# IrisRainbowNeko/HCP-Diffusion

Measured on AMD Instinct MI355X. Metric: training images/sec (whole node), SD1.5 LoRA 512px bs=4/GPU, higher is better.
Workload: dtype bf16; 1 GPU; SD1.5 UNet LoRA rank=8 bf16, bs=4/GPU, 512x512 (64x64 latents), 77-token context, random-init weights, cached latents, grad-ckpt off; global_batch=4, parallelism=dp1, rccl_ranks=1, comm=none, hip_graph=True, gradient_checkpointing=False

## Files before the change

hcp_diffusion_amd/csrc/gemm.hip:

```cpp
#include "hcp_common.h"
#include "gemm_params.h"

extern "C" int hcp_geglu_fwd(const void* h, void* y, long M, int F, hipStream_t stream);

namespace {

using namespace hcp_gemm;


HCP_DEVICE void epilogue_store(const GemmParams& p, int m, int n, hcp_f32x4 v) {
    if (p.geglu_hg) { epilogue_geglu_bwd(p, m, n, v); return; }
    v = v * p.alpha;
    if (p.bias) v += *(const hcp_f32x4*)(p.bias + n);
    if (p.rowbias) v += *(const hcp_f32x4*)(p.rowbias + (size_t)(m / p.rows_per_group) * p.rowbias_ld + n);
    if (p.residual) {
        hcp_bf16x4 r = *(const hcp_bf16x4*)(p.residual + (size_t)m * p.ldr + n);
#pragma unroll
        for (int q = 0; q < 4; ++q) v[q] += hcp_bf2f((unsigned short)r[q]);
        add_residual_lo(p, m, n, v);
    }
    if (p.out_f32) *(hcp_f32x4*)((float*)p.D + (size_t)m * p.ldd + n) = v;
    else store_hi_lo(p, m, n, v);
}

// ... 744 lines not shown
            const hcp_f32x4 a = *(const hcp_f32x4*)(src + (size_t)s * slab), b = *(const hcp_f32x4*)(src + (size_t)(s + 1) * slab);
            v += a; v += b;
            s += 2;
        }
        if (s < ns) v += *(const hcp_f32x4*)(src + (size_t)s * slab);
        if (!plain) { epilogue_geglu_bwd(p, m, n, v); continue; }
        v = v * p.alpha;
        if (p.bias) v += bias;
        if (p.rowbias) v += rowb;
        if (p.residual) {
#pragma unroll
            for (int q = 0; q < 4; ++q) v[q] += hcp_bf2f((unsigned short)res[q]);
            if (p.residual_lo) {
#pragma unroll
                for (int q = 0; q < 4; ++q) v[q] += hcp_bf2f((unsigned short)res_lo[q]);
            }
        }
        if (p.out_f32) *(hcp_f32x4*)((float*)p.D + (size_t)m * p.ldd + n) = v;
        else store_hi_lo(p, m, n, v);
    }
}

HCP_TUNABLE(int, g_force_cfg, -1);
HCP_TUNABLE(int, g_dbg_ablate, 0);
HCP_TUNABLE(int, g_use_glds, 1);
HCP_TUNABLE(int, g_use_v2, 1);

HCP_TUNABLE(int, g_conv_patch, 1);
HCP_TUNABLE(int, g_epi_tile, -1);
HCP_TUNABLE(int, g_force_loaders, -1);

bool want_epi_tile(const GemmParams& p, int mode) {
    if (p.nsplit != 1 || p.out_f32 || p.geglu_hg || p.geglu_out || p.N % 8 || p.ldd % 8 || (p.residual && p.ldr % 8)) return false;
    if ((((size_t)p.D) | ((size_t)p.D_lo) | ((size_t)p.residual) | ((size_t)p.residual_lo)) & 15) return false;
    if (g_epi_tile >= 0) return g_epi_tile == 1;
    return mode == 0 && p.residual != nullptr;
}

template <int BM, int BN, int WGM, int WGN, int MODE, bool FAST, bool LORA = false, int NSTAGE = 2, int NLD = 0>
int launch_cfg(GemmParams& p, hipStream_t stream) {
    p.tiles_m = hcp_cdiv(p.M, BM);
    const int tiles_n = hcp_cdiv(p.N, BN);
    p.dbg = g_dbg_ablate;
    if constexpr (NSTAGE == 2 && (MODE == 0 || FAST)) {
        if (g_use_v2 && g_use_glds && !(p.dbg & 7) && p.K % BK == 0 && (p.K2 == 0 || p.K2 == 32) &&
            (size_t)p.M * p.lda * 2 < (1ul << 31) && (size_t)p.N * p.ldb * 2 < (1ul << 31)) {
// ... 32 lines not shown
            HCP_LAUNCH_CHECK("gemm_v2_kernel");
        }
    }
    {
        p.epi_tile = 0;
        p.geglu_out = nullptr;
        size_t smem = (size_t)NSTAGE * (BM + BN + (LORA ? 32 : 0)) * BK * sizeof(hcp_bf16);
        const size_t tail = (size_t)(2 * BM + BN) * 40 * sizeof(hcp_bf16);
        if (LORA && smem < tail) smem = tail;
        HCP_LAUNCH((gemm_glds_kernel<BM, BN, WGM, WGN, MODE, FAST, LORA, NSTAGE>), dim3(p.tiles_m * tiles_n, p.nsplit),
                   dim3(64 * WGM * WGN), smem, stream, p);
    }
    if (p.nsplit > 1) {
        long nv = (long)p.M * (p.N / 4);
        int g = (int)((nv + 255) / 256); if (g > 2048) g = 2048;
        HCP_LAUNCH(splitk_reduce_kernel, dim3(g), dim3(256), 0, stream, p);
    }
    HCP_LAUNCH_CHECK("gemm_kernel");
}

struct TileCfg { int bm, bn; };
constexpr TileCfg kCfgs[] = {{128, 128}, {128, 64}, {64, 64}, {128, 160}, {64, 160}, {256, 128}, {256, 160}, {128, 320},
                             {128, 160}, {128, 160}, {256, 160},
                             {128, 320}, {256, 160}, {128, 160}, {64, 160}, {128, 128}};
constexpr int kNumCfgs = sizeof(kCfgs) / sizeof(kCfgs[0]);

int try_pp(int id, int mode, bool fast_or_plain, bool lora, GemmParams& p, hipStream_t stream) {
    if (p.loaders < 8 || !fast_or_plain || !g_use_v2 || (g_dbg_ablate & 7)) return -2;
    if (p.K % BK != 0 || !(p.K2 == 0 || p.K2 == 32) || (size_t)p.M * p.lda * 2 >= (1ul << 31) || (size_t)p.N * p.ldb * 2 >= (1ul << 31)) return -2;
    const int bm = kCfgs[id].bm, bn = kCfgs[id].bn;
    p.tiles_m = hcp_cdiv(p.M, bm);
    p.dbg = g_dbg_ablate;
    p.epi_tile = want_epi_tile(p, mode) ? 1 : 0;
    hcp_bf16* const gout = p.geglu_out;
    if (gout) {
        if (mode == 0 && p.nsplit == 1 && (p.N / 2) % (bn / 2) == 0) p.geglu_fused = 1;
        else p.geglu_out = nullptr;
    }
    int r = -2;
    if (mode != 0 && !lora && (g_conv_patch == 2 || (g_conv_patch == 1 && (mode == 2 || p.nsplit > 1))))
        r = conv_patch_launch(p, bm, bn, mode, p.loaders - 8, stream);
    if (r == -2) r = gemm_pp_launch(p, bm, bn, mode, lora, p.loaders - 8, stream);
    if (r == -2) { p.geglu_out = gout; p.geglu_fused = 0; }
    if (r != 0 || p.nsplit <= 1) return r;
    long nv = (long)p.M * (p.N / 4);
    int g = (int)((nv + 255) / 256); if (g > 2048) g = 2048;
    HCP_LAUNCH(splitk_reduce_kernel, dim3(g), dim3(256), 0, stream, p);
    HCP_LAUNCH_CHECK("splitk_reduce_kernel");
}

template <int MODE, bool FAST>
int launch_by_id(int id, GemmParams& p, hipStream_t stream) {
    if (id >= 0 && id < kNumCfgs) { const int r = try_pp(id, MODE, MODE == 0 || FAST, false, p, stream); if (r != -2) return r; }
    switch (id) {
        case 0: return launch_cfg<128, 128, 2, 2, MODE, FAST>(p, stream);
        case 1: return launch_cfg<128, 64, 2, 2, MODE, FAST>(p, stream);
        case 2: return launch_cfg<64, 64, 2, 2, MODE, FAST>(p, stream);
        case 3: return launch_cfg<128, 160, 2, 2, MODE, FAST>(p, stream);
        case 4: return launch_cfg<64, 160, 2, 2, MODE, FAST>(p, stream);
        case 5: return launch_cfg<256, 128, 4, 2, MODE, FAST>(p, stream);
        case 6: return launch_cfg<256, 160, 4, 2, MODE, FAST>(p, stream);
        case 8: return launch_cfg<128, 160, 4, 2, MODE, FAST, false, 3>(p, stream);
        case 9: return launch_cfg<128, 160, 2, 2, MODE, FAST, false, 3>(p, stream);
        case 10: return launch_cfg<256, 160, 4, 2, MODE, FAST, false, 3>(p, stream);
        case 11: return launch_cfg<128, 320, 4, 4, MODE, FAST>(p, stream);
        case 12: return launch_cfg<256, 160, 8, 2, MODE, FAST>(p, stream);
        case 13: return launch_cfg<128, 160, 4, 2, MODE, FAST, false, 2, 4>(p, stream);
        case 14: return launch_cfg<64, 160, 4, 2, MODE, FAST, false, 2, 4>(p, stream);
        case 15: return launch_cfg<128, 128, 4, 2, MODE, FAST, false, 2, 4>(p, stream);
        default: return launch_cfg<128, 320, 2, 4, MODE, FAST>(p, stream);
    }
}

int launch_lora_by_id(int id, GemmParams& p, hipStream_t stream) {
    if (id >= 0 && id < kNumCfgs) { const int r = try_pp(id, 0, true, true, p, stream); if (r != -2) return r; }
    switch (id) {
        case 0: return launch_cfg<128, 128, 2, 2, 0, false, true>(p, stream);
        case 1: return launch_cfg<128, 64, 2, 2, 0, false, true>(p, stream);
        case 2: return launch_cfg<64, 64, 2, 2, 0, false, true>(p, stream);
        case 3: return launch_cfg<128, 160, 2, 2, 0, false, true>(p, stream);
        case 5: return launch_cfg<256, 128, 4, 2, 0, false, true>(p, stream);
        case 6: return launch_cfg<256, 160, 4, 2, 0, false, true>(p, stream);
        case 8: return launch_cfg<128, 160, 4, 2, 0, false, true, 3>(p, stream);
        case 9: return launch_cfg<128, 160, 2, 2, 0, false, true, 3>(p, stream);
        case 12: return launch_cfg<256, 160, 8, 2, 0, false, true>(p, stream);
        case 13: return launch_cfg<128, 160, 4, 2, 0, false, true, 2, 4>(p, stream);
        case 14: return launch_cfg<64, 160, 4, 2, 0, false, true, 2, 4>(p, stream);
        case 15: return launch_cfg<128, 128, 4, 2, 0, false, true, 2, 4>(p, stream);
        default: return launch_cfg<64, 160, 2, 2, 0, false, true>(p, stream);
    }
}

int choose_cfg(const GemmParams& p, int* nsplit_out) {
    const int nk1 = hcp_cdiv(p.K, BK);
    int id;
    if (p.N <= 64) id = 2;
    else if (p.N % 160 == 0) id = ((long)p.M * p.N >= (long)4096 * 2560) ? 6 : 4;
    else id = ((long)p.M * p.N >= (long)4096 * 2048) ? 0 : 2;
    const long tiles = (long)hcp_cdiv(p.M, kCfgs[id].bm) * hcp_cdiv(p.N, kCfgs[id].bn);
    int s = 1;
    while (s < 16 && tiles * s < 1024 && nk1 / (s * 2) >= 4) s *= 2;
    *nsplit_out = s;
    return id;
}

struct TunedEntry { int mode, M, N, K, has_k2, stride, up, cfg, split, loaders; };
const TunedEntry kTuned[] = {
#include "gemm_tuned_loaders.inc"
#include "gemm_tuned.inc"
};

// ... 3 lines not shown

bool lookup_tuned(const GemmParams& p, int mode, int* cfg, int* split, int* loaders = nullptr) {
    bool hit = false;
    for (const TunedEntry& e : kTuned) {
        if (g_force_loaders == 0 && e.loaders) continue;
        if (e.mode == mode && e.M == p.M && e.N == p.N && e.K == p.K && e.has_k2 == (p.K2 > 0) &&
            (mode == 0 || mode == 3 || (e.stride == p.cv.stride && e.up == p.cv.up))) {
            *cfg = e.cfg; *split = e.split; if (loaders) *loaders = e.loaders; hit = true; break;
        }
    }
#if defined(HCP_TOOLS)
    (hit ? g_table_hits : g_table_misses) += 1;
#endif
    return hit;
}

inline int deepest_ring(int ld) { return ld == 3 ? 4 : ld; }

template <int MODE, bool FAST>
int dispatch_gemm(GemmParams& p, float* ws, size_t ws_bytes, hipStream_t stream) {
    int nsplit = 1;
    int id = 0, ld = 0;
    if (!lookup_tuned(p, MODE, &id, &nsplit, &ld)) id = choose_cfg(p, &nsplit);
    if (g_force_cfg >= 0) { id = g_force_cfg % 16; nsplit = g_force_cfg / 16 > 0 ? g_force_cfg / 16 : 1; }
    p.loaders = g_force_loaders >= 0 ? g_force_loaders : deepest_ring(ld);
    if (nsplit > 1 && (size_t)nsplit * p.M * p.N * sizeof(float) > ws_bytes) nsplit = 1;
    if (p.geglu_out) nsplit = 1;
    const int nk1 = hcp_cdiv(p.K, BK);
    p.nsplit = nsplit;
    p.kt_per_split = hcp_cdiv(nk1, nsplit);
    p.nsplit = hcp_cdiv(nk1, p.kt_per_split);
    p.slabs = ws;
    return launch_by_id<MODE, FAST>(id, p, stream);
}

int check_common(const GemmParams& p) {
    HCP_REQUIRE(p.M > 0 && p.N > 0 && p.K > 0, "gemm: empty problem M=%d N=%d K=%d", p.M, p.N, p.K);
    HCP_REQUIRE(p.K % 8 == 0 && p.K2 % 8 == 0, "gemm: K (%d) and K2 (%d) must be multiples of 8", p.K, p.K2);
    HCP_REQUIRE(p.N % 4 == 0 && p.ldd % 4 == 0, "gemm: N (%d) and ldd (%d) must be multiples of 4", p.N, p.ldd);
    HCP_REQUIRE(p.ldb % 8 == 0, "gemm: ldb (%d) must be a multiple of 8", p.ldb);
    HCP_REQUIRE(p.K2 == 0 || (p.A2 && p.B2 && p.lda2 % 8 == 0 && p.ldb2 % 8 == 0), "gemm: bad K-extension operands");
    HCP_REQUIRE(!p.residual || p.ldr % 4 == 0, "gemm: ldr must be a multiple of 4");
    HCP_REQUIRE(!p.rowbias || p.rows_per_group > 0, "gemm: rows_per_group must be > 0");
    return 0;
}

int check_gact(GemmParams& p, void* gact, const char* who) {
    if (!gact) return 0;
    HCP_REQUIRE(!p.out_f32 && !p.residual && !p.rowbias && !p.D_lo && p.alpha == 1.0f && p.N % 16 == 0 && p.ldd == p.N,
                "%s: the GEGLU output needs a contiguous bf16 (h | g) [M, N] (N %% 16 == 0) with no residual / row bias / alpha", who);
    p.geglu_out = (hcp_bf16*)gact; p.geglu_fused = 0;
    return 0;
}
int finish_gact(const GemmParams& p, void* gact, hipStream_t stream) {
    if (!gact || p.geglu_fused) return 0;
    return hcp_geglu_fwd(p.D, gact, p.M, p.N / 2, stream);
}

int launch_lora_dispatched(GemmParams& p, void* workspace, size_t workspace_bytes, hipStream_t stream) {
    int id = 4, nsplit = 1, ld = 0;
    GemmParams q = p; q.K2 = 32;
    if (!lookup_tuned(q, 3, &id, &nsplit, &ld)) {
        if (p.K >= 4096 && p.M <= 4096) id = -1;
        else if ((long)p.M * p.N >= (long)4096 * 2560 && p.N % 160 == 0) id = 6;
        else if (p.N % 160 == 0 && (long)p.M * p.N >= (long)4096 * 640) id = 4;
        else id = 2;
    }
    if (g_force_cfg >= 0) id = g_force_cfg % 16;
    p.loaders = g_force_loaders >= 0 ? g_force_loaders : deepest_ring(ld);
    if (id == 7 || id == 10 || id == 11) id = 6;
    if (id < 0) {
        HCP_REQUIRE(p.Tout, "hcp_gemm_lora_bf16: this shape runs as two launches and needs the T buffer");
        const int ldt = p.ldt == 64 ? 64 : 32;
        if (ldt == 64 && hcp_memset_async(p.Tout, 0, (size_t)p.M * 64 * sizeof(hcp_bf16), stream)) return hcp_set_error("hcp_gemm_lora_bf16: memset failed");
        GemmParams t = {};
        t.A = p.A; t.lda = p.lda; t.B = p.L; t.ldb = p.K; t.M = p.M; t.N = 32; t.K = p.K; t.D = p.Tout; t.ldd = ldt; t.alpha = 1.0f;
        if (int e2 = dispatch_gemm<0, false>(t, (float*)workspace, workspace ? workspace_bytes : 0, stream)) return e2;
        p.A2 = (const hcp_bf16*)p.Tout; p.lda2 = ldt; p.B2 = p.E; p.ldb2 = 32; p.K2 = 32;
        p.L = nullptr; p.E = nullptr; p.Tout = nullptr; p.ldt = 0;
        return dispatch_gemm<0, false>(p, (float*)workspace, workspace ? workspace_bytes : 0, stream);
    }
    p.nsplit = 1; p.kt_per_split = hcp_cdiv(p.K, BK); p.slabs = nullptr;
    return launch_lora_by_id(id, p, stream);
}

}

#if defined(HCP_TOOLS)
HCP_API int hcp_debug_gemm_table_stats(long* hits, long* misses) {
    if (hits) *hits = g_table_hits;
    if (misses) *misses = g_table_misses;
// ... 99 lines not shown
```

hcp_diffusion_amd/csrc/gemm_pp.hip:

```cpp
#include "gemm_params.h"
#include <type_traits>

namespace hcp_gemm {
namespace {

template <int BM, int BN, int MODE, bool LORA, int NST>
HCP_KERNEL(768) gemm_pp_kernel(GemmParams p) {
    constexpr int NC = 8, NLD = 4;
    constexpr int NTC = 64 * NC, NTL = 64 * NLD;
    constexpr int WTM = BM / 2, WTN = BN / 2;
    constexpr int TM = WTM / 16, TN = WTN / 16;
    constexpr int UPT = 1;
    constexpr int TMF = TM / 2;
    constexpr int RPP = NTL / 8;
    constexpr int A_IT = BM / RPP, B_IT = BN / RPP;
    static_assert(WTM % 16 == 0 && WTN % 16 == 0 && BM % RPP == 0 && BN % RPP == 0 && TM % 2 == 0, "tile shape");
    static_assert(NST >= 2 && NST <= 4, "ring depth");
    constexpr int A_ELEMS = BM * BK, B_ELEMS = BN * BK, L_ELEMS = LORA ? 32 * BK : 0, BUF_ELEMS = A_ELEMS + B_ELEMS + L_ELEMS;
    constexpr int E_ELEMS = LORA ? BN * 32 : 0;
    HCP_DYN_SMEM(smem);
    hcp_bf16* const lds_e = (hcp_bf16*)smem;
    hcp_bf16* const ring = lds_e + E_ELEMS;

    const int tid_all = threadIdx.x;
    const int lane = tid_all & 63;
    const int wave_all = hcp_uniform(tid_all >> 6);
    const int tile_m = blockIdx.x % p.tiles_m, tile_n = blockIdx.x / p.tiles_m;
    const int m0 = tile_m * BM, n0 = tile_n * BN;
    const int split = blockIdx.y;

    const int nk1 = p.K / BK;
    const int kt_begin = split * p.kt_per_split;
    int kt_end = kt_begin + p.kt_per_split; if (kt_end > nk1) kt_end = nk1;
    const int nprim = kt_end - kt_begin;
    const bool has_ext = (split == p.nsplit - 1) && p.K2 > 0;
    const int nk = nprim + (has_ext ? 1 : 0);

    if (wave_all >= NC) {
        const int wave = wave_all - NC, tid = tid_all - NTC;
// ... 182 lines not shown
                } else {
                    issue_part(I0{}, std::integral_constant<int, IPT / 4>{}, wbuf, ext);
                    hcp_barrier_only();
                    issue_part(std::integral_constant<int, IPT / 4>{}, std::integral_constant<int, IPT / 2>{}, wbuf, ext);
                    hcp_barrier_only();
                    issue_part(std::integral_constant<int, IPT / 2>{}, std::integral_constant<int, LASTQ>{}, wbuf, ext);
                }
                hcp_wait_vmcnt_c<(NST - 3) * IPT + LASTQ>();
                hcp_barrier_only();
                issue_part(std::integral_constant<int, LASTQ>{}, IALL{}, wbuf, ext); tile_done();
            }
        }
        for (; t < nk; ++t) quiet_iter(t);
        hcp_barrier_only();
        hcp_barrier_only(); hcp_barrier_only();
        if (LORA) HCP_SYNC();
        if ((p.geglu_hg || p.geglu_out || p.epi_tile) && p.nsplit == 1) { if (LORA) HCP_SYNC(); HCP_SYNC(); }
        return;
    }

    const int g = wave_all >> 2, gm = (wave_all >> 1) & 1, gn = wave_all & 1;
    const int fr = lane & 15, fg = lane >> 4;
    const int row0 = gm * WTM;
    const int frow0 = gm * WTM + g * (WTM / 2);
    const int col0 = gn * WTN;
    const int sw0 = ((fg ^ ((fr >> 1) & 7)) << 3) ^ (g * 32);
    const int a_rd0 = (row0 + fr) * BK + sw0;
    const int b_rd0 = A_ELEMS + (col0 + fr) * BK + sw0;
    const int l_rd0 = A_ELEMS + B_ELEMS + (gn * 16 + fr) * BK + sw0;

    hcp_f32x4 acc[TM][TN];
    hcp_f32x4 tacc[LORA ? TM : 1];
#pragma unroll
    for (int i = 0; i < TM; ++i)
#pragma unroll
        for (int j = 0; j < TN; ++j) { hcp_f32x4 z = {0.f, 0.f, 0.f, 0.f}; acc[i][j] = z; }
#pragma unroll
    for (int i = 0; i < (LORA ? TM : 1); ++i) { hcp_f32x4 z = {0.f, 0.f, 0.f, 0.f}; tacc[i] = z; }

    constexpr bool EARLY = !(LORA && TM * TN >= 20);
    hcp_f32x4 bias_v[TN];
    hcp_bf16x4 res_v[TMF][TN];
    auto load_bias = [&]() {
        const hcp_rsrc rbias = hcp_make_rsrc_n(p.bias, p.bias ? (unsigned)p.N * 4u : 0u);
#pragma unroll
        for (int j = 0; j < TN; ++j) bias_v[j] = hcp_buf_load16f(rbias, (unsigned)geglu_col(p, BN, n0 + col0 + j * 16 + 4 * fg) * 4u);
    };
    auto load_residual = [&]() {
        const hcp_rsrc rres = hcp_make_rsrc_n(p.residual, p.residual ? (unsigned)(((size_t)(p.M - 1) * p.ldr + p.N) * 2) : 0u);
#pragma unroll
        for (int i = 0; i < TMF; ++i) {
            const int m = m0 + frow0 + i * 16 + fr;
#pragma unroll
            for (int j = 0; j < TN; ++j)
                res_v[i][j] = hcp_buf_load8(rres, ((unsigned)m * (unsigned)p.ldr + (unsigned)(n0 + col0 + j * 16 + 4 * fg)) * 2u);
        }
    };

    if (EARLY && p.nsplit == 1 && !p.epi_tile) load_residual();
    hcp_barrier_only();
    if (g == 1) hcp_barrier_only();
    for (int t = 0, st = 0; t < nk; ++t) {
        const hcp_bf16* sp = ring + st * BUF_ELEMS;
#pragma unroll
        for (int u = 0; u < UPT; ++u) {
#if defined(HCP_TOOLS)
            if (p.dbg & 0x800) { hcp_barrier_only(); hcp_barrier_only(); continue; }
#endif
            hcp_bf16x8 fa[TM], fb[TN], fl;
            constexpr int x = 0;
#pragma unroll
            for (int i = 0; i < TM; ++i) fa[i] = *(const hcp_bf16x8*)(sp + (a_rd0 ^ x) + i * 16 * BK);
#pragma unroll
            for (int j = 0; j < TN; ++j) fb[j] = *(const hcp_bf16x8*)(sp + (b_rd0 ^ x) + j * 16 * BK);
            if (LORA) fl = *(const hcp_bf16x8*)(sp + (l_rd0 ^ x));
            hcp_barrier_only();
#if defined(HCP_TOOLS)
            if (p.dbg & 0x400) {
// ... 4 lines not shown
                hcp_barrier_only();
                continue;
            }
#endif
#if defined(HCP_TOOLS)
            if (!(p.dbg & 0x1000))
#endif
            hcp_setprio<1>();
#pragma unroll
            for (int i = 0; i < TM; ++i)
#pragma unroll
                for (int j = 0; j < TN; ++j) acc[i][j] = hcp_mfma16(fb[j], fa[i], acc[i][j]);
            if (LORA) {
#pragma unroll
                for (int i = 0; i < TM; ++i) tacc[i] = hcp_mfma16(fl, fa[i], tacc[i]);
            }
            hcp_setprio<0>();
            hcp_barrier_only();
        }
        st = st + 1 == NST ? 0 : st + 1;
    }
    if (g == 0) hcp_barrier_only();

    if (g == 1) {
#pragma unroll
        for (int i = 0; i < TMF; ++i) {
#pragma unroll
            for (int j = 0; j < TN; ++j) { const hcp_f32x4 tmp = acc[i][j]; acc[i][j] = acc[TMF + i][j]; acc[TMF + i][j] = tmp; }
            if (LORA) { const hcp_f32x4 tmp = tacc[i]; tacc[i] = tacc[TMF + i]; tacc[TMF + i] = tmp; }
        }
    }
    {
        hcp_f32x4* const xb = (hcp_f32x4*)ring;
        hcp_f32x4* const xt = xb + NC * TMF * TN * 64;
#pragma unroll
        for (int i = 0; i < TMF; ++i) {
#pragma unroll
            for (int j = 0; j < TN; ++j) xb[((wave_all * TMF + i) * TN + j) * 64 + lane] = acc[TMF + i][j];
            if (LORA) xt[(wave_all * TMF + i) * 64 + lane] = tacc[TMF + i];
        }
        if (p.nsplit == 1) load_bias();
        hcp_barrier_keep_dma();
        const int pw = wave_all ^ 4;
#pragma unroll
        for (int i = 0; i < TMF; ++i) {
#pragma unroll
            for (int j = 0; j < TN; ++j) acc[i][j] += xb[((pw * TMF + i) * TN + j) * 64 + lane];
            if (LORA) tacc[i] += xt[(pw * TMF + i) * 64 + lane];
        }
        hcp_barrier_keep_dma();
    }

    if (LORA) {
        constexpr int TS2 = 40;
        hcp_bf16* lt = ring;
        hcp_bf16* lt2 = ring + BM * TS2;
        const bool split = p.ldt == 64;
        const int ldt = split ? 64 : 32;
#pragma unroll
        for (int i = 0; i < TMF; ++i) {
            hcp_bf16x4 o, o2;
            lora_t_split(tacc[i], o, o2);
            const int ml = frow0 + i * 16 + fr;
            *(hcp_bf16x4*)(lt + ml * TS2 + gn * 16 + 4 * fg) = o;
            if (split) *(hcp_bf16x4*)(lt2 + ml * TS2 + gn * 16 + 4 * fg) = o2;
            if (tile_n == 0 && p.Tout && m0 + ml < p.M) {
                *(hcp_bf16x4*)(p.Tout + (size_t)(m0 + ml) * ldt + gn * 16 + 4 * fg) = o;
                if (split) *(hcp_bf16x4*)(p.Tout + (size_t)(m0 + ml) * ldt + 32 + gn * 16 + 4 * fg) = o2;
            }
        }
        if (!EARLY && p.nsplit == 1 && !p.epi_tile) load_residual();
        HCP_SYNC();
        hcp_bf16x8 ft[TMF], fe[TN];
#pragma unroll
        for (int i = 0; i < TMF; ++i) ft[i] = *(const hcp_bf16x8*)(lt + (frow0 + i * 16 + fr) * TS2 + fg * 8);
#pragma unroll
        for (int j = 0; j < TN; ++j) fe[j] = *(const hcp_bf16x8*)(lds_e + (col0 + j * 16 + fr) * 32 + fg * 8);
#pragma unroll
        for (int i = 0; i < TMF; ++i)
#pragma unroll
            for (int j = 0; j < TN; ++j) acc[i][j] = hcp_mfma16(fe[j], ft[i], acc[i][j]);
        if (split) {
#pragma unroll
            for (int i = 0; i < TMF; ++i) ft[i] = *(const hcp_bf16x8*)(lt2 + (frow0 + i * 16 + fr) * TS2 + fg * 8);
#pragma unroll
            for (int i = 0; i < TMF; ++i)
#pragma unroll
                for (int j = 0; j < TN; ++j) acc[i][j] = hcp_mfma16(fe[j], ft[i], acc[i][j]);
        }
    }

    if (p.nsplit > 1) {
#pragma unroll
        for (int i = 0; i < TMF; ++i) {
            const int m = m0 + frow0 + i * 16 + fr;
            if (m >= p.M) continue;
#pragma unroll
            for (int j = 0; j < TN; ++j) {
                const int n = n0 + col0 + j * 16 + 4 * fg;
                if (n < p.N) *(hcp_f32x4*)(p.slabs + ((size_t)split * p.M + m) * p.N + n) = acc[i][j];
            }
        }
        return;
    }
    if (p.geglu_hg) {
        if (LORA) HCP_SYNC();
#pragma unroll
        for (int i = 0; i < TMF; ++i)
#pragma unroll
            for (int j = 0; j < TN; ++j) geglu_tile_put(ring, geglu_tile_ld(BN), frow0 + i * 16 + fr, col0 + j * 16 + 4 * fg, acc[i][j], p.alpha);
        HCP_SYNC();
        geglu_tile_apply<BM, BN, NTC>(p, ring, m0, n0, tid_all);
        return;
    }
    if (p.geglu_out) {
        static_assert((size_t)BM * BN * 2 <= (size_t)NST * BUF_ELEMS * sizeof(hcp_bf16), "the gelu(g) tile fits the ring");
        if (LORA) HCP_SYNC();
        hcp_f32x4 v[TMF][TN];
        int rows[TMF], cols[TN];
        const bool is_g = gn == 1;
#pragma unroll
        for (int j = 0; j < TN; ++j) cols[j] = tile_n * (BN / 2) + j * 16 + 4 * fg;
#pragma unroll
        for (int i = 0; i < TMF; ++i) {
            const int m = m0 + frow0 + i * 16 + fr;
            rows[i] = m;
#pragma unroll
            for (int j = 0; j < TN; ++j) {
                v[i][j] = acc[i][j] * p.alpha + bias_v[j];
                if (m < p.M) store_hi_lo(p, m, cols[j] + (is_g ? (p.N >> 1) : 0), v[i][j]);
            }
        }
        geglu_fwd_pair<TMF, TN>(v, is_g, wave_all >> 1, lane, (hcp_f32x4*)ring, [] { HCP_SYNC(); }, p.geglu_out, p.N >> 1, rows, p.M, cols);
        return;
    }
    if (p.epi_tile) {
        if (LORA) HCP_SYNC();
        float* const tile = (float*)ring;
#pragma unroll
        for (int i = 0; i < TMF; ++i) {
            const int ml = frow0 + i * 16 + fr, m = m0 + ml;
            const float* rbp = (p.rowbias && m < p.M) ? p.rowbias + (size_t)(m / p.rows_per_group) * p.rowbias_ld : nullptr;
#pragma unroll
            for (int j = 0; j < TN; ++j) {
                const int nl = col0 + j * 16 + 4 * fg;
                hcp_f32x4 v = acc[i][j] * p.alpha + bias_v[j];
                if (rbp && n0 + nl < p.N) v += *(const hcp_f32x4*)(rbp + n0 + nl);
                *(hcp_f32x4*)(tile + ml * epi_tile_ld(BN) + nl) = v;
            }
        }
        HCP_SYNC();
        epi_tile_store<BM, BN, NTC>(p, tile, m0, n0, tid_all);
        return;
    }
#pragma unroll
    for (int i = 0; i < TMF; ++i) {
        const int m = m0 + frow0 + i * 16 + fr;
        if (m >= p.M) continue;
        hcp_f32x4 rb_v[TN];
        if (p.rowbias) {
            const float* rbp = p.rowbias + (size_t)(m / p.rows_per_group) * p.rowbias_ld;
#pragma unroll
            for (int j = 0; j < TN; ++j) {
                const int n = n0 + col0 + j * 16 + 4 * fg;
                hcp_f32x4 z = {0.f, 0.f, 0.f, 0.f};
                rb_v[j] = n < p.N ? *(const hcp_f32x4*)(rbp + n) : z;
            }
        }
#pragma unroll
        for (int j = 0; j < TN; ++j) {
            const int n = n0 + col0 + j * 16 + 4 * fg;
            if (n >= p.N) continue;
            hcp_f32x4 v = acc[i][j] * p.alpha + bias_v[j];
            if (p.rowbias) v += rb_v[j];
            if (p.residual) {
#pragma unroll
                for (int q = 0; q < 4; ++q) v[q] += hcp_bf2f((unsigned short)res_v[i][j][q]);
                add_residual_lo(p, m, n, v);
            }
            if (p.out_f32) *(hcp_f32x4*)((float*)p.D + (size_t)m * p.ldd + n) = v;
            else store_hi_lo(p, m, n, v);
        }
    }
}

template <int BM, int BN, int MODE, bool LORA>
int launch_pp(GemmParams& p, int ring, hipStream_t stream) {
    constexpr size_t stage = (size_t)(BM + BN + (LORA ? 32 : 0)) * BK * sizeof(hcp_bf16);
    constexpr size_t eimg = LORA ? (size_t)BN * 32 * sizeof(hcp_bf16) : 0;
    constexpr int TMF = BM / 64;
    constexpr size_t xchg = (size_t)8 * TMF * (BN / 32) * 64 * 16 + (LORA ? (size_t)8 * TMF * 64 * 16 : 0);
    constexpr size_t tail = LORA ? (size_t)2 * BM * 40 * sizeof(hcp_bf16) : 0;
    constexpr size_t tile_bytes = (size_t)BM * epi_tile_ld(BN) * sizeof(float);
    if (p.epi_tile && tile_bytes + eimg > 160 * 1024) p.epi_tile = 0;
    const size_t floor_ = (xchg > tail ? xchg : tail) > (p.epi_tile ? tile_bytes : 0) ? (xchg > tail ? xchg : tail) : tile_bytes;
    constexpr size_t cap = 160 * 1024;
    const dim3 grid(p.tiles_m * hcp_cdiv(p.N, BN), p.nsplit);
    if (ring >= 4 && 4 * stage + eimg <= cap) {
        constexpr int R = 4 * stage + eimg <= cap ? 4 : 2;
        const size_t sm = (R * stage > floor_ ? R * stage : floor_) + eimg;
        HCP_LAUNCH((gemm_pp_kernel<BM, BN, MODE, LORA, R>), grid, dim3(768), sm, stream, p);
    } else if (ring >= 3 && 3 * stage + eimg <= cap) {
        constexpr int R = 3 * stage + eimg <= cap ? 3 : 2;
        const size_t sm = (R * stage > floor_ ? R * stage : floor_) + eimg;
        HCP_LAUNCH((gemm_pp_kernel<BM, BN, MODE, LORA, R>), grid, dim3(768), sm, stream, p);
    } else {
        const size_t sm = (2 * stage > floor_ ? 2 * stage : floor_) + eimg;
        HCP_LAUNCH((gemm_pp_kernel<BM, BN, MODE, LORA, 2>), grid, dim3(768), sm, stream, p);
    }
    HCP_LAUNCH_CHECK("gemm_pp_kernel");
}

template <int BM, int BN>
int launch_pp_mode(GemmParams& p, int mode, bool lora, int ring, hipStream_t stream) {
    if (lora) return launch_pp<BM, BN, 0, true>(p, ring, stream);
    if (mode == 0) return launch_pp<BM, BN, 0, false>(p, ring, stream);
    if (mode == 1) return launch_pp<BM, BN, 1, false>(p, ring, stream);
    return launch_pp<BM, BN, 2, false>(p, ring, stream);
}

}

int gemm_pp_launch(GemmParams& p, int bm, int bn, int mode, bool lora, int ring, hipStream_t stream) {
    if (p.residual && (size_t)p.M * p.ldr * 2 >= (1ul << 31)) return -2;
    if (bm == 128 && bn == 160) return launch_pp_mode<128, 160>(p, mode, lora, ring, stream);
    if (bm == 64 && bn == 160) return launch_pp_mode<64, 160>(p, mode, lora, ring, stream);
    if (bm == 128 && bn == 128) return launch_pp_mode<128, 128>(p, mode, lora, ring, stream);
    return -2;
}

}
```

hcp_diffusion_amd/csrc/gemm_tuned_loaders.inc:

```
{3, 4096, 640, 640, 1, 1, 0, 14, 1, 11},
{3, 1024, 1280, 1280, 1, 1, 0, 14, 1, 12},
{0, 4096, 640, 640, 0, 1, 0, 14, 1, 11},
{0, 1024, 1280, 1280, 0, 1, 0, 14, 1, 11},
{2, 256, 1280, 11520, 0, 1, 0, 15, 8, 12},
{1, 16384, 320, 2880, 0, 1, 0, 13, 1, 12},
{1, 4096, 640, 5760, 0, 1, 0, 13, 2, 12},
{2, 4096, 640, 5760, 0, 1, 0, 13, 2, 11},
{3, 4096, 640, 2560, 1, 1, 0, 14, 1, 12},
{3, 1024, 1280, 5120, 1, 1, 0, 14, 1, 12},
{2, 16384, 320, 2880, 0, 1, 0, 13, 1, 12},
{3, 4096, 640, 5120, 1, 1, 0, 14, 1, 12},
{3, 4096, 640, 1920, 1, 1, 0, 14, 1, 12},
{3, 1024, 1280, 3840, 1, 1, 0, 14, 1, 12},
{0, 256, 1280, 1280, 0, 1, 0, 14, 1, 11},
{0, 256, 1280, 2560, 0, 1, 0, 14, 4, 12},
{0, 256, 2560, 1280, 0, 1, 0, 14, 1, 11},
{0, 1024, 1280, 2560, 0, 1, 0, 14, 2, 12},
{1, 16384, 320, 5760, 0, 1, 0, 13, 1, 12},
{2, 1024, 2560, 11520, 0, 1, 0, 13, 2, 12},
{0, 4, 1280, 1280, 0, 1, 0, 14, 4, 11},
{0, 4, 20160, 1280, 0, 1, 0, 14, 1, 12},
{1, 4096, 640, 2880, 0, 1, 0, 14, 1, 12},
{1, 1024, 1280, 5760, 0, 1, 0, 14, 2, 12},
{0, 1024, 1280, 640, 0, 1, 0, 14, 1, 11},
{1, 256, 1280, 11520, 0, 2, 0, 15, 8, 12},
{3, 256, 3840, 1280, 1, 1, 0, 14, 1, 12},
{0, 1024, 1280, 1920, 0, 1, 0, 14, 1, 12},
{1, 4096, 640, 17280, 0, 1, 0, 13, 2, 12},
{0, 4096, 640, 1920, 0, 1, 0, 14, 1, 12},
{1, 4096, 640, 11520, 0, 1, 0, 13, 2, 12},
{0, 4096, 640, 1280, 0, 1, 0, 14, 1, 11},
{1, 4096, 640, 8640, 0, 1, 0, 13, 2, 12},
{0, 4096, 640, 960, 0, 1, 0, 14, 1, 11},
{1, 16384, 320, 8640, 0, 1, 0, 13, 8, 12},
{0, 16384, 320, 960, 0, 1, 0, 13, 1, 12},
{2, 16384, 960, 2880, 0, 1, 0, 13, 8, 12},
{2, 4096, 960, 5760, 0, 1, 0, 15, 1, 12},
{2, 4096, 1280, 5760, 0, 1, 0, 13, 1, 11},
{2, 4096, 1920, 5760, 0, 1, 0, 15, 1, 12},
{2, 4096, 1280, 11520, 0, 1, 0, 13, 8, 12},
{2, 1024, 1920, 11520, 0, 1, 0, 15, 2, 12},
{3, 256, 5120, 1280, 1, 1, 0, 14, 1, 12},
{0, 1024, 640, 1280, 0, 1, 0, 14, 1, 11},
{2, 1024, 640, 11520, 0, 1, 0, 14, 4, 12},
{0, 4096, 320, 640, 0, 1, 0, 14, 1, 11},
{2, 4096, 320, 5760, 0, 1, 0, 13, 4, 11},
{0, 16384, 32, 960, 0, 1, 0, 14, 1, 12},
{0, 308, 512, 24960, 0, 1, 0, 15, 8, 12},
{3, 2048, 1280, 1280, 1, 1, 0, 14, 1, 12},
{3, 2048, 1280, 5120, 1, 1, 0, 14, 1, 12},
{3, 2048, 1280, 10240, 1, 1, 0, 14, 1, 12},
{3, 2048, 1280, 2560, 1, 1, 0, 14, 1, 12},
{0, 2048, 1280, 1280, 0, 1, 0, 14, 1, 12},
{1, 2048, 1280, 11520, 0, 1, 0, 13, 2, 12},
{2, 2048, 1280, 11520, 0, 1, 0, 13, 2, 12},
{1, 8192, 640, 5760, 0, 1, 0, 13, 8, 12},
{2, 8192, 640, 5760, 0, 1, 0, 13, 1, 12},
{0, 2, 1280, 1280, 0, 1, 0, 14, 4, 11},
{1, 2048, 1280, 23040, 0, 1, 0, 13, 2, 12},
{0, 2048, 1280, 2560, 0, 1, 0, 14, 1, 12},
{0, 2048, 2560, 1280, 0, 1, 0, 13, 1, 12},
{2, 2048, 2560, 11520, 0, 1, 0, 13, 8, 12},
{0, 2, 1280, 320, 0, 1, 0, 14, 1, 11},
{0, 2, 1280, 2816, 0, 1, 0, 14, 8, 11},
{0, 2, 13760, 1280, 0, 1, 0, 14, 2, 12},
{1, 8192, 320, 2880, 0, 2, 0, 14, 1, 12},
{1, 8192, 640, 2880, 0, 1, 0, 13, 1, 12},
{1, 2048, 640, 5760, 0, 2, 0, 13, 4, 11},
// ... 97 lines not shown
{2, 2048, 960, 5760, 0, 1, 0, 13, 2, 3},
{2, 2048, 1280, 5760, 0, 1, 0, 13, 2, 3},
{0, 2048, 1920, 640, 0, 1, 0, 15, 1, 3},
{2, 2048, 1920, 5760, 0, 1, 0, 13, 1, 3},
{0, 512, 1920, 1280, 0, 1, 0, 15, 1, 3},
{2, 512, 1920, 11520, 0, 1, 0, 15, 4, 3},
{0, 128, 5120, 1280, 0, 1, 0, 14, 1, 3},
{0, 128, 1280, 10240, 0, 1, 0, 14, 8, 4},
{2, 512, 1280, 11520, 0, 2, 0, 13, 8, 3},
{0, 512, 640, 1280, 0, 1, 0, 14, 1, 3},
{2, 512, 640, 11520, 0, 1, 0, 15, 8, 3},
{2, 2048, 640, 5760, 0, 2, 0, 13, 8, 4},
{2, 2048, 320, 5760, 0, 1, 0, 14, 4, 3},
{2, 8192, 320, 2880, 0, 2, 0, 13, 4, 1},
{3, 2048, 2560, 1280, 1, 1, 0, 13, 1, 3},
{3, 16384, 320, 320, 1, 1, 0, 13, 1, 3},
{3, 308, 640, 768, 1, 1, 0, 13, 1, 1},
{3, 16384, 320, 1280, 1, 1, 0, 13, 1, 3},
{3, 1024, 3840, 1280, 1, 1, 0, 15, 1, 3},
{3, 16384, 320, 2560, 1, 1, 0, 13, 1, 3},
{0, 308, 32, 640, 0, 1, 0, 14, 1, 4},
{3, 1024, 5120, 1280, 1, 1, 0, 13, 1, 3},
{3, 16384, 320, 960, 1, 1, 0, 13, 1, 3},
{0, 4, 1280, 320, 0, 1, 0, 15, 1, 1},
{0, 4096, 640, 320, 0, 1, 0, 14, 1, 3},
{3, 256, 10240, 1280, 1, 1, 0, 15, 1, 3},
{1, 16384, 4, 2880, 0, 1, 0, 15, 2, 4},
{3, 8192, 640, 640, 1, 1, 0, 13, 1, 3},
{3, 154, 2560, 2048, 1, 1, 0, 14, 1, 4},
{0, 154, 32, 2560, 0, 1, 0, 13, 4, 4},
{0, 8192, 640, 640, 0, 1, 0, 13, 1, 3},
{3, 8192, 640, 2560, 1, 1, 0, 13, 1, 3},
{3, 8192, 640, 5120, 1, 1, 0, 13, 1, 3},
{0, 154, 32, 1280, 0, 1, 0, 14, 1, 4},
{0, 8192, 640, 1280, 0, 1, 0, 13, 1, 3},
{0, 8192, 640, 960, 0, 1, 0, 13, 1, 3},
{0, 8192, 960, 640, 0, 1, 0, 15, 1, 3},
{0, 8192, 1280, 640, 0, 1, 0, 13, 1, 4},
{0, 2048, 1920, 1280, 0, 1, 0, 15, 1, 4},
{2, 8192, 640, 5760, 0, 2, 0, 13, 2, 3},
```

Measured before the change: 205.6 images/sec.

## Add 32-row GEMM tile with N-split cross-wave reduction and retune small-M shapes

Adds a BM=32, BN=160 tile config (id 16) to the pipelined GEMM kernel. With only one 16-row MFMA fragment per wave, the two wave groups now split the finalisation across N columns instead of M rows when exchanging and reducing partial accumulators. The tuned table moves many small-M shapes (M=4, 256, 1024, 308) to this config and bumps loader ring settings, aiming for more workgroups and better CU occupancy on skinny GEMMs. In exchange, each tile gets less data reuse and the new finalisation path is more complex. Geglu fused output is not supported for this tile.

New measurement: 209.4 images/sec, median of 6. 1.9% higher.

```diff
diff --git a/hcp_diffusion_amd/csrc/gemm.hip b/hcp_diffusion_amd/csrc/gemm.hip
--- a/hcp_diffusion_amd/csrc/gemm.hip
+++ b/hcp_diffusion_amd/csrc/gemm.hip
@@ -790,6 +790,8 @@
 }
 
 HCP_TUNABLE(int, g_force_cfg, -1);
+inline int forced_id(int v) { return v >= 1024 ? (v - 1024) % 64 : v % 16; }
+inline int forced_split(int v) { const int s = v >= 1024 ? (v - 1024) / 64 : v / 16; return s > 0 ? s : 1; }
 HCP_TUNABLE(int, g_dbg_ablate, 0);
 HCP_TUNABLE(int, g_use_glds, 1);
 HCP_TUNABLE(int, g_use_v2, 1);
@@ -868,7 +870,8 @@
 struct TileCfg { int bm, bn; };
 constexpr TileCfg kCfgs[] = {{128, 128}, {128, 64}, {64, 64}, {128, 160}, {64, 160}, {256, 128}, {256, 160}, {128, 320},
                              {128, 160}, {128, 160}, {256, 160},
-                             {128, 320}, {256, 160}, {128, 160}, {64, 160}, {128, 128}};
+                             {128, 320}, {256, 160}, {128, 160}, {64, 160}, {128, 128},
+                             {32, 160}};
 constexpr int kNumCfgs = sizeof(kCfgs) / sizeof(kCfgs[0]);
 
 int try_pp(int id, int mode, bool fast_or_plain, bool lora, GemmParams& p, hipStream_t stream) {
@@ -914,6 +917,7 @@
         case 13: return launch_cfg<128, 160, 4, 2, MODE, FAST, false, 2, 4>(p, stream);
         case 14: return launch_cfg<64, 160, 4, 2, MODE, FAST, false, 2, 4>(p, stream);
         case 15: return launch_cfg<128, 128, 4, 2, MODE, FAST, false, 2, 4>(p, stream);
+        case 16: return launch_cfg<64, 160, 4, 2, MODE, FAST, false, 2, 4>(p, stream);
         default: return launch_cfg<128, 320, 2, 4, MODE, FAST>(p, stream);
     }
 }
@@ -933,6 +937,7 @@
         case 13: return launch_cfg<128, 160, 4, 2, 0, false, true, 2, 4>(p, stream);
         case 14: return launch_cfg<64, 160, 4, 2, 0, false, true, 2, 4>(p, stream);
         case 15: return launch_cfg<128, 128, 4, 2, 0, false, true, 2, 4>(p, stream);
+        case 16: return launch_cfg<64, 160, 4, 2, 0, false, true, 2, 4>(p, stream);
         default: return launch_cfg<64, 160, 2, 2, 0, false, true>(p, stream);
     }
 }
@@ -982,7 +987,7 @@
     int nsplit = 1;
     int id = 0, ld = 0;
     if (!lookup_tuned(p, MODE, &id, &nsplit, &ld)) id = choose_cfg(p, &nsplit);
-    if (g_force_cfg >= 0) { id = g_force_cfg % 16; nsplit = g_force_cfg / 16 > 0 ? g_force_cfg / 16 : 1; }
+    if (g_force_cfg >= 0) { id = forced_id(g_force_cfg); nsplit = forced_split(g_force_cfg); }
     p.loaders = g_force_loaders >= 0 ? g_force_loaders : deepest_ring(ld);
     if (nsplit > 1 && (size_t)nsplit * p.M * p.N * sizeof(float) > ws_bytes) nsplit = 1;
     if (p.geglu_out) nsplit = 1;
@@ -1026,7 +1031,7 @@
         else if (p.N % 160 == 0 && (long)p.M * p.N >= (long)4096 * 640) id = 4;
         else id = 2;
     }
-    if (g_force_cfg >= 0) id = g_force_cfg % 16;
+    if (g_force_cfg >= 0) id = forced_id(g_force_cfg);
     p.loaders = g_force_loaders >= 0 ? g_force_loaders : deepest_ring(ld);
     if (id == 7 || id == 10 || id == 11) id = 6;
     if (id < 0) {
diff --git a/hcp_diffusion_amd/csrc/gemm_pp.hip b/hcp_diffusion_amd/csrc/gemm_pp.hip
--- a/hcp_diffusion_amd/csrc/gemm_pp.hip
+++ b/hcp_diffusion_amd/csrc/gemm_pp.hip
@@ -11,10 +11,13 @@
     constexpr int WTM = BM / 2, WTN = BN / 2;
     constexpr int TM = WTM / 16, TN = WTN / 16;
     constexpr int UPT = 1;
-    constexpr int TMF = TM / 2;
+    constexpr bool FIN_N = TM == 1;
+    constexpr int TMF = FIN_N ? 1 : TM / 2;
+    constexpr int TNF0 = FIN_N ? (TN + 1) / 2 : TN, TNF1 = FIN_N ? TN / 2 : TN;
+    constexpr int TNF = TNF0;
     constexpr int RPP = NTL / 8;
     constexpr int A_IT = BM / RPP, B_IT = BN / RPP;
-    static_assert(WTM % 16 == 0 && WTN % 16 == 0 && BM % RPP == 0 && BN % RPP == 0 && TM % 2 == 0, "tile shape");
+    static_assert(WTM % 16 == 0 && WTN % 16 == 0 && BM % RPP == 0 && BN % RPP == 0 && (TM % 2 == 0 || FIN_N), "tile shape");
     static_assert(NST >= 2 && NST <= 4, "ring depth");
     constexpr int A_ELEMS = BM * BK, B_ELEMS = BN * BK, L_ELEMS = LORA ? 32 * BK : 0, BUF_ELEMS = A_ELEMS + B_ELEMS + L_ELEMS;
     constexpr int E_ELEMS = LORA ? BN * 32 : 0;
@@ -243,8 +246,10 @@
     const int g = wave_all >> 2, gm = (wave_all >> 1) & 1, gn = wave_all & 1;
     const int fr = lane & 15, fg = lane >> 4;
     const int row0 = gm * WTM;
-    const int frow0 = gm * WTM + g * (WTM / 2);
+    const int frow0 = FIN_N ? row0 : gm * WTM + g * (WTM / 2);
     const int col0 = gn * WTN;
+    const int fcol0 = col0 + (FIN_N ? g * TNF0 * 16 : 0);
+    const int nfin = FIN_N && g == 1 ? TNF1 : TNF0;
     const int sw0 = ((fg ^ ((fr >> 1) & 7)) << 3) ^ (g * 32);
     const int a_rd0 = (row0 + fr) * BK + sw0;
     const int b_rd0 = A_ELEMS + (col0 + fr) * BK + sw0;
@@ -260,12 +265,12 @@
     for (int i = 0; i < (LORA ? TM : 1); ++i) { hcp_f32x4 z = {0.f, 0.f, 0.f, 0.f}; tacc[i] = z; }
 
     constexpr bool EARLY = !(LORA && TM * TN >= 20);
-    hcp_f32x4 bias_v[TN];
-    hcp_bf16x4 res_v[TMF][TN];
+    hcp_f32x4 bias_v[TNF];
+    hcp_bf16x4 res_v[TMF][TNF];
     auto load_bias = [&]() {
         const hcp_rsrc rbias = hcp_make_rsrc_n(p.bias, p.bias ? (unsigned)p.N * 4u : 0u);
 #pragma unroll
-        for (int j = 0; j < TN; ++j) bias_v[j] = hcp_buf_load16f(rbias, (unsigned)geglu_col(p, BN, n0 + col0 + j * 16 + 4 * fg) * 4u);
+        for (int j = 0; j < TNF; ++j) bias_v[j] = hcp_buf_load16f(rbias, (unsigned)geglu_col(p, BN, n0 + fcol0 + j * 16 + 4 * fg) * 4u);
     };
     auto load_residual = [&]() {
         const hcp_rsrc rres = hcp_make_rsrc_n(p.residual, p.residual ? (unsigned)(((size_t)(p.M - 1) * p.ldr + p.N) * 2) : 0u);
@@ -273,8 +278,8 @@
         for (int i = 0; i < TMF; ++i) {
             const int m = m0 + frow0 + i * 16 + fr;
 #pragma unroll
-            for (int j = 0; j < TN; ++j)
-                res_v[i][j] = hcp_buf_load8(rres, ((unsigned)m * (unsigned)p.ldr + (unsigned)(n0 + col0 + j * 16 + 4 * fg)) * 2u);
+            for (int j = 0; j < TNF; ++j)
+                res_v[i][j] = hcp_buf_load8(rres, ((unsigned)m * (unsigned)p.ldr + (unsigned)(n0 + fcol0 + j * 16 + 4 * fg)) * 2u);
         }
     };
 
@@ -325,17 +330,44 @@
     }
     if (g == 0) hcp_barrier_only();
 
-    if (g == 1) {
-#pragma unroll
-        for (int i = 0; i < TMF; ++i) {
-#pragma unroll
-            for (int j = 0; j < TN; ++j) { const hcp_f32x4 tmp = acc[i][j]; acc[i][j] = acc[TMF + i][j]; acc[TMF + i][j] = tmp; }
-            if (LORA) { const hcp_f32x4 tmp = tacc[i]; tacc[i] = tacc[TMF + i]; tacc[TMF + i] = tmp; }
-        }
-    }
-    {
-        hcp_f32x4* const xb = (hcp_f32x4*)ring;
-        hcp_f32x4* const xt = xb + NC * TMF * TN * 64;
+    hcp_f32x4* const xb = (hcp_f32x4*)ring;
+    hcp_f32x4* const xt = xb + NC * TMF * (FIN_N ? TNF0 : TN) * 64;
+    const int pw = wave_all ^ 4;
+    if constexpr (FIN_N) {
+        if (g == 1) {
+            hcp_f32x4 tmp[TN];
+#pragma unroll
+            for (int j = 0; j < TN; ++j) tmp[j] = acc[0][j];
+#pragma unroll
+            for (int j = 0; j < TN; ++j) acc[0][j] = tmp[(j + TNF0) % TN];
+        }
+        if (g == 0) {
+#pragma unroll
+            for (int k = 0; k < TNF1; ++k) xb[(wave_all * TNF0 + k) * 64 + lane] = acc[0][TNF0 + k];
+        } else {
+#pragma unroll
+            for (int k = 0; k < TNF0; ++k) xb[(wave_all * TNF0 + k) * 64 + lane] = acc[0][TNF1 + k];
+            if (LORA) xt[wave_all * 64 + lane] = tacc[0];
+        }
+        if (p.nsplit == 1) load_bias();
+        hcp_barrier_keep_dma();
+        if (g == 0) {
+#pragma unroll
+            for (int k = 0; k < TNF0; ++k) acc[0][k] += xb[(pw * TNF0 + k) * 64 + lane];
+            if (LORA) tacc[0] += xt[pw * 64 + lane];
+        } else {
+#pragma unroll
+            for (int k = 0; k < TNF1; ++k) acc[0][k] += xb[(pw * TNF0 + k) * 64 + lane];
+        }
+    } else {
+        if (g == 1) {
+#pragma unroll
+            for (int i = 0; i < TMF; ++i) {
+#pragma unroll
+                for (int j = 0; j < TN; ++j) { const hcp_f32x4 tmp = acc[i][j]; acc[i][j] = acc[TMF + i][j]; acc[TMF + i][j] = tmp; }
+                if (LORA) { const hcp_f32x4 tmp = tacc[i]; tacc[i] = tacc[TMF + i]; tacc[TMF + i] = tmp; }
+            }
+        }
 #pragma unroll
         for (int i = 0; i < TMF; ++i) {
 #pragma unroll
@@ -344,15 +376,14 @@
         }
         if (p.nsplit == 1) load_bias();
         hcp_barrier_keep_dma();
-        const int pw = wave_all ^ 4;
 #pragma unroll
         for (int i = 0; i < TMF; ++i) {
 #pragma unroll
             for (int j = 0; j < TN; ++j) acc[i][j] += xb[((pw * TMF + i) * TN + j) * 64 + lane];
             if (LORA) tacc[i] += xt[(pw * TMF + i) * 64 + lane];
         }
-        hcp_barrier_keep_dma();
-    }
+    }
+    hcp_barrier_keep_dma();
 
     if (LORA) {
         constexpr int TS2 = 40;
@@ -362,6 +393,7 @@
         const int ldt = split ? 64 : 32;
 #pragma unroll
         for (int i = 0; i < TMF; ++i) {
+            if (FIN_N && g == 1) break;
             hcp_bf16x4 o, o2;
             lora_t_split(tacc[i], o, o2);
             const int ml = frow0 + i * 16 + fr;
@@ -374,22 +406,22 @@
         }
         if (!EARLY && p.nsplit == 1 && !p.epi_tile) load_residual();
         HCP_SYNC();
-        hcp_bf16x8 ft[TMF], fe[TN];
+        hcp_bf16x8 ft[TMF], fe[TNF];
 #pragma unroll
         for (int i = 0; i < TMF; ++i) ft[i] = *(const hcp_bf16x8*)(lt + (frow0 + i * 16 + fr) * TS2 + fg * 8);
 #pragma unroll
-        for (int j = 0; j < TN; ++j) fe[j] = *(const hcp_bf16x8*)(lds_e + (col0 + j * 16 + fr) * 32 + fg * 8);
+        for (int j = 0; j < TNF; ++j) fe[j] = *(const hcp_bf16x8*)(lds_e + (fcol0 + j * 16 + fr) * 32 + fg * 8);
 #pragma unroll
         for (int i = 0; i < TMF; ++i)
 #pragma unroll
-            for (int j = 0; j < TN; ++j) acc[i][j] = hcp_mfma16(fe[j], ft[i], acc[i][j]);
+            for (int j = 0; j < TNF; ++j) acc[i][j] = hcp_mfma16(fe[j], ft[i], acc[i][j]);
         if (split) {
 #pragma unroll
             for (int i = 0; i < TMF; ++i) ft[i] = *(const hcp_bf16x8*)(lt2 + (frow0 + i * 16 + fr) * TS2 + fg * 8);
 #pragma unroll
             for (int i = 0; i < TMF; ++i)
 #pragma unroll
-                for (int j = 0; j < TN; ++j) acc[i][j] = hcp_mfma16(fe[j], ft[i], acc[i][j]);
+                for (int j = 0; j < TNF; ++j) acc[i][j] = hcp_mfma16(fe[j], ft[i], acc[i][j]);
         }
     }
 
@@ -399,9 +431,9 @@
             const int m = m0 + frow0 + i * 16 + fr;
             if (m >= p.M) continue;
 #pragma unroll
-            for (int j = 0; j < TN; ++j) {
-                const int n = n0 + col0 + j * 16 + 4 * fg;
-                if (n < p.N) *(hcp_f32x4*)(p.slabs + ((size_t)split * p.M + m) * p.N + n) = acc[i][j];
+            for (int j = 0; j < TNF; ++j) {
+                const int n = n0 + fcol0 + j * 16 + 4 * fg;
+                if (j < nfin && n < p.N) *(hcp_f32x4*)(p.slabs + ((size_t)split * p.M + m) * p.N + n) = acc[i][j];
             }
         }
         return;
@@ -411,12 +443,13 @@
 #pragma unroll
         for (int i = 0; i < TMF; ++i)
 #pragma unroll
-            for (int j = 0; j < TN; ++j) geglu_tile_put(ring, geglu_tile_ld(BN), frow0 + i * 16 + fr, col0 + j * 16 + 4 * fg, acc[i][j], p.alpha);
+            for (int j = 0; j < TNF; ++j)
+                if (j < nfin) geglu_tile_put(ring, geglu_tile_ld(BN), frow0 + i * 16 + fr, fcol0 + j * 16 + 4 * fg, acc[i][j], p.alpha);
         HCP_SYNC();
         geglu_tile_apply<BM, BN, NTC>(p, ring, m0, n0, tid_all);
         return;
     }
-    if (p.geglu_out) {
+    if constexpr (!FIN_N) if (p.geglu_out) {
         static_assert((size_t)BM * BN * 2 <= (size_t)NST * BUF_ELEMS * sizeof(hcp_bf16), "the gelu(g) tile fits the ring");
         if (LORA) HCP_SYNC();
         hcp_f32x4 v[TMF][TN];
@@ -445,8 +478,9 @@
             const int ml = frow0 + i * 16 + fr, m = m0 + ml;
             const float* rbp = (p.rowbias && m < p.M) ? p.rowbias + (size_t)(m / p.rows_per_group) * p.rowbias_ld : nullptr;
 #pragma unroll
-            for (int j = 0; j < TN; ++j) {
-                const int nl = col0 + j * 16 + 4 * fg;
+            for (int j = 0; j < TNF; ++j) {
+                if (j >= nfin) continue;
+                const int nl = fcol0 + j * 16 + 4 * fg;
                 hcp_f32x4 v = acc[i][j] * p.alpha + bias_v[j];
                 if (rbp && n0 + nl < p.N) v += *(const hcp_f32x4*)(rbp + n0 + nl);
                 *(hcp_f32x4*)(tile + ml * epi_tile_ld(BN) + nl) = v;
@@ -460,20 +494,20 @@
     for (int i = 0; i < TMF; ++i) {
         const int m = m0 + frow0 + i * 16 + fr;
         if (m >= p.M) continue;
-        hcp_f32x4 rb_v[TN];
+        hcp_f32x4 rb_v[TNF];
         if (p.rowbias) {
             const float* rbp = p.rowbias + (size_t)(m / p.rows_per_group) * p.rowbias_ld;
 #pragma unroll
-            for (int j = 0; j < TN; ++j) {
-                const int n = n0 + col0 + j * 16 + 4 * fg;
+            for (int j = 0; j < TNF; ++j) {
+                const int n = n0 + fcol0 + j * 16 + 4 * fg;
                 hcp_f32x4 z = {0.f, 0.f, 0.f, 0.f};
                 rb_v[j] = n < p.N ? *(const hcp_f32x4*)(rbp + n) : z;
             }
         }
 #pragma unroll
-        for (int j = 0; j < TN; ++j) {
-            const int n = n0 + col0 + j * 16 + 4 * fg;
-            if (n >= p.N) continue;
+        for (int j = 0; j < TNF; ++j) {
+            const int n = n0 + fcol0 + j * 16 + 4 * fg;
+            if (j >= nfin || n >= p.N) continue;
             hcp_f32x4 v = acc[i][j] * p.alpha + bias_v[j];
             if (p.rowbias) v += rb_v[j];
             if (p.residual) {
@@ -491,8 +525,9 @@
 int launch_pp(GemmParams& p, int ring, hipStream_t stream) {
     constexpr size_t stage = (size_t)(BM + BN + (LORA ? 32 : 0)) * BK * sizeof(hcp_bf16);
     constexpr size_t eimg = LORA ? (size_t)BN * 32 * sizeof(hcp_bf16) : 0;
-    constexpr int TMF = BM / 64;
-    constexpr size_t xchg = (size_t)8 * TMF * (BN / 32) * 64 * 16 + (LORA ? (size_t)8 * TMF * 64 * 16 : 0);
+    constexpr int TM = BM / 32, TN = BN / 32;
+    constexpr int TMF = TM == 1 ? 1 : TM / 2, TNX = TM == 1 ? (TN + 1) / 2 : TN;
+    constexpr size_t xchg = (size_t)8 * TMF * TNX * 64 * 16 + (LORA ? (size_t)8 * TMF * 64 * 16 : 0);
     constexpr size_t tail = LORA ? (size_t)2 * BM * 40 * sizeof(hcp_bf16) : 0;
     constexpr size_t tile_bytes = (size_t)BM * epi_tile_ld(BN) * sizeof(float);
     if (p.epi_tile && tile_bytes + eimg > 160 * 1024) p.epi_tile = 0;
@@ -528,6 +563,10 @@
     if (p.residual && (size_t)p.M * p.ldr * 2 >= (1ul << 31)) return -2;
     if (bm == 128 && bn == 160) return launch_pp_mode<128, 160>(p, mode, lora, ring, stream);
     if (bm == 64 && bn == 160) return launch_pp_mode<64, 160>(p, mode, lora, ring, stream);
+    if (bm == 32 && bn == 160) {
+        if (mode != 0 || p.geglu_out) return -2;
+        return lora ? launch_pp<32, 160, 0, true>(p, ring, stream) : launch_pp<32, 160, 0, false>(p, ring, stream);
+    }
     if (bm == 128 && bn == 128) return launch_pp_mode<128, 128>(p, mode, lora, ring, stream);
     return -2;
 }
diff --git a/hcp_diffusion_amd/csrc/gemm_tuned_loaders.inc b/hcp_diffusion_amd/csrc/gemm_tuned_loaders.inc
--- a/hcp_diffusion_amd/csrc/gemm_tuned_loaders.inc
+++ b/hcp_diffusion_amd/csrc/gemm_tuned_loaders.inc
@@ -1,37 +1,44 @@
-{3, 4096, 640, 640, 1, 1, 0, 14, 1, 11},
-{3, 1024, 1280, 1280, 1, 1, 0, 14, 1, 12},
-{0, 4096, 640, 640, 0, 1, 0, 14, 1, 11},
-{0, 1024, 1280, 1280, 0, 1, 0, 14, 1, 11},
+{3, 4096, 640, 640, 1, 1, 0, 14, 1, 12},
+{3, 1024, 1280, 1280, 1, 1, 0, 16, 1, 12},
+{0, 4096, 640, 640, 0, 1, 0, 14, 1, 12},
+{0, 1024, 1280, 1280, 0, 1, 0, 16, 1, 12},
+{3, 256, 1280, 1280, 1, 1, 0, 16, 2, 12},
+{3, 4096, 1920, 640, 1, 1, 0, 14, 1, 12},
+{3, 1024, 1280, 5120, 1, 1, 0, 16, 4, 12},
+{3, 1024, 1280, 3840, 1, 1, 0, 16, 4, 12},
+{0, 256, 1280, 1280, 0, 1, 0, 16, 4, 12},
+{0, 256, 1280, 2560, 0, 1, 0, 16, 4, 12},
+{0, 256, 2560, 1280, 0, 1, 0, 16, 1, 12},
+{0, 4, 1280, 320, 0, 1, 0, 16, 1, 12},
+{0, 4, 1280, 1280, 0, 1, 0, 16, 4, 12},
+{0, 4, 20160, 1280, 0, 1, 0, 16, 2, 12},
+{0, 308, 512, 768, 0, 1, 0, 16, 1, 12},
+{0, 1024, 1280, 640, 0, 1, 0, 16, 1, 12},
+{3, 256, 3840, 1280, 1, 1, 0, 16, 1, 12},
+{3, 256, 10240, 1280, 1, 1, 0, 14, 2, 12},
+{0, 1024, 1280, 1920, 0, 1, 0, 16, 1, 12},
+{0, 4096, 640, 1280, 0, 1, 0, 14, 1, 12},
+{0, 4096, 640, 960, 0, 1, 0, 14, 1, 12},
+{0, 1024, 640, 1280, 0, 1, 0, 16, 1, 12},
+{0, 4096, 320, 640, 0, 1, 0, 16, 1, 12},
 {2, 256, 1280, 11520, 0, 1, 0, 15, 8, 12},
 {1, 16384, 320, 2880, 0, 1, 0, 13, 1, 12},
 {1, 4096, 640, 5760, 0, 1, 0, 13, 2, 12},
 {2, 4096, 640, 5760, 0, 1, 0, 13, 2, 11},
 {3, 4096, 640, 2560, 1, 1, 0, 14, 1, 12},
-{3, 1024, 1280, 5120, 1, 1, 0, 14, 1, 12},
 {2, 16384, 320, 2880, 0, 1, 0, 13, 1, 12},
 {3, 4096, 640, 5120, 1, 1, 0, 14, 1, 12},
 {3, 4096, 640, 1920, 1, 1, 0, 14, 1, 12},
-{3, 1024, 1280, 3840, 1, 1, 0, 14, 1, 12},
-{0, 256, 1280, 1280, 0, 1, 0, 14, 1, 11},
-{0, 256, 1280, 2560, 0, 1, 0, 14, 4, 12},
-{0, 256, 2560, 1280, 0, 1, 0, 14, 1, 11},
 {0, 1024, 1280, 2560, 0, 1, 0, 14, 2, 12},
 {1, 16384, 320, 5760, 0, 1, 0, 13, 1, 12},
 {2, 1024, 2560, 11520, 0, 1, 0, 13, 2, 12},
-{0, 4, 1280, 1280, 0, 1, 0, 14, 4, 11},
-{0, 4, 20160, 1280, 0, 1, 0, 14, 1, 12},
 {1, 4096, 640, 2880, 0, 1, 0, 14, 1, 12},
 {1, 1024, 1280, 5760, 0, 1, 0, 14, 2, 12},
-{0, 1024, 1280, 640, 0, 1, 0, 14, 1, 11},
 {1, 256, 1280, 11520, 0, 2, 0, 15, 8, 12},
-{3, 256, 3840, 1280, 1, 1, 0, 14, 1, 12},
-{0, 1024, 1280, 1920, 0, 1, 0, 14, 1, 12},
 {1, 4096, 640, 17280, 0, 1, 0, 13, 2, 12},
 {0, 4096, 640, 1920, 0, 1, 0, 14, 1, 12},
 {1, 4096, 640, 11520, 0, 1, 0, 13, 2, 12},
-{0, 4096, 640, 1280, 0, 1, 0, 14, 1, 11},
 {1, 4096, 640, 8640, 0, 1, 0, 13, 2, 12},
-{0, 4096, 640, 960, 0, 1, 0, 14, 1, 11},
 {1, 16384, 320, 8640, 0, 1, 0, 13, 8, 12},
 {0, 16384, 320, 960, 0, 1, 0, 13, 1, 12},
 {2, 16384, 960, 2880, 0, 1, 0, 13, 8, 12},
@@ -41,9 +48,7 @@
 {2, 4096, 1280, 11520, 0, 1, 0, 13, 8, 12},
 {2, 1024, 1920, 11520, 0, 1, 0, 15, 2, 12},
 {3, 256, 5120, 1280, 1, 1, 0, 14, 1, 12},
-{0, 1024, 640, 1280, 0, 1, 0, 14, 1, 11},
 {2, 1024, 640, 11520, 0, 1, 0, 14, 4, 12},
-{0, 4096, 320, 640, 0, 1, 0, 14, 1, 11},
 {2, 4096, 320, 5760, 0, 1, 0, 13, 4, 11},
 {0, 16384, 32, 960, 0, 1, 0, 14, 1, 12},
 {0, 308, 512, 24960, 0, 1, 0, 15, 8, 12},
@@ -187,9 +192,7 @@
 {0, 308, 32, 640, 0, 1, 0, 14, 1, 4},
 {3, 1024, 5120, 1280, 1, 1, 0, 13, 1, 3},
 {3, 16384, 320, 960, 1, 1, 0, 13, 1, 3},
-{0, 4, 1280, 320, 0, 1, 0, 15, 1, 1},
 {0, 4096, 640, 320, 0, 1, 0, 14, 1, 3},
-{3, 256, 10240, 1280, 1, 1, 0, 15, 1, 3},
 {1, 16384, 4, 2880, 0, 1, 0, 15, 2, 4},
 {3, 8192, 640, 640, 1, 1, 0, 13, 1, 3},
 {3, 154, 2560, 2048, 1, 1, 0, 14, 1, 4},
```
